# gduguey/DiffUS

Measured on NVIDIA B200. Metric: bmode_frames_per_s_fwd_bwd, higher is better.
Workload: dtype f32

## Files before the change

### diffus_b200/csrc/common.cuh

```cuda
#pragma once
#include <cuda_runtime.h>
#include <stdint.h>
#include <float.h>

#include "../../include/diffus_b200.h"

namespace diffus {

constexpr unsigned FULL = 0xffffffffu;

template <int CH, int CK = 2>
struct Geo {
    static constexpr int CHUNK = CH;
    static constexpr int CKPT = CK;
    static constexpr int SEG = 32 * CH;
    __device__ __forceinline__ static int pad(int i) { return i + (i >> 5); }
    static constexpr int ZBUF = (SEG + 2) + (SEG + 2) / 32 + 3;
    static constexpr int OBUF = (SEG + 1) + (SEG + 1) / 32 + 3;
};
using FwdGeo = Geo<16>;
using BwdGeo = Geo<8, 2>;
constexpr int PREFIX_STRIDE = FwdGeo::SEG;

struct M2 {
    float2 c0, c1;
    __device__ __forceinline__ float a() const { return c0.x; }
    __device__ __forceinline__ float b() const { return c1.x; }
    __device__ __forceinline__ float c() const { return c0.y; }
    __device__ __forceinline__ float d() const { return c1.y; }
};
__device__ __forceinline__ float2 bcast(float s) { return make_float2(s, s); }
__device__ __forceinline__ M2 m2_make(float a, float b, float c, float d) { return M2{make_float2(a, c), make_float2(b, d)}; }
__device__ __forceinline__ M2 m2_identity() { return m2_make(1.f, 0.f, 0.f, 1.f); }
__device__ __forceinline__ M2 m2_zero() { return m2_make(0.f, 0.f, 0.f, 0.f); }
__device__ __forceinline__ M2 m2_mul(const M2& x, const M2& y) {
    return M2{__ffma2_rn(x.c0, bcast(y.c0.x), __fmul2_rn(x.c1, bcast(y.c0.y))),
              __ffma2_rn(x.c0, bcast(y.c1.x), __fmul2_rn(x.c1, bcast(y.c1.y)))};
}
__device__ __forceinline__ M2 m2_mul_interface(const M2& p, float r) {
    float q = __fmaf_rn(-2.f * r, r, 1.f);
    return M2{__ffma2_rn(p.c0, bcast(q), __fmul2_rn(p.c1, bcast(-r))), __ffma2_rn(p.c0, bcast(r), p.c1)};
}
__device__ __forceinline__ M2 m2_mul_interface_t(const M2& x, float r) {
    float q = __fmaf_rn(-2.f * r, r, 1.f);
    return M2{__ffma2_rn(x.c0, bcast(q), __fmul2_rn(x.c1, bcast(r))), __ffma2_rn(x.c0, bcast(-r), x.c1)};
}
__device__ __forceinline__ M2 m2_transpose(const M2& x) { return m2_make(x.a(), x.c(), x.b(), x.d()); }
__device__ __forceinline__ M2 m2_add(const M2& x, const M2& y) { return M2{__fadd2_rn(x.c0, y.c0), __fadd2_rn(x.c1, y.c1)}; }
__device__ __forceinline__ float2 shfl_up2(float2 v, int d) { return make_float2(__shfl_up_sync(FULL, v.x, d), __shfl_up_sync(FULL, v.y, d)); }
__device__ __forceinline__ float2 shfl_down2(float2 v, int d) { return make_float2(__shfl_down_sync(FULL, v.x, d), __shfl_down_sync(FULL, v.y, d)); }
__device__ __forceinline__ float2 shfl2(float2 v, int src) { return make_float2(__shfl_sync(FULL, v.x, src), __shfl_sync(FULL, v.y, src)); }
__device__ __forceinline__ M2 m2_shfl_up(const M2& x, int d) { return M2{shfl_up2(x.c0, d), shfl_up2(x.c1, d)}; }
__device__ __forceinline__ M2 m2_shfl_down(const M2& x, int d) { return M2{shfl_down2(x.c0, d), shfl_down2(x.c1, d)}; }
__device__ __forceinline__ M2 m2_shfl(const M2& x, int src) { return M2{shfl2(x.c0, src), shfl2(x.c1, src)}; }

__device__ __forceinline__ float nan_to_num(float e) {
    if (e != e) return 0.f;
    return fminf(fmaxf(e, -FLT_MAX), FLT_MAX);
}

__device__ __forceinline__ float warp_sum(float v) {
#pragma unroll
    for (int d = 16; d > 0; d >>= 1) v += __shfl_xor_sync(FULL, v, d);
    return v;
}

__device__ __forceinline__ int warp_sum8_index(int lane) { return ((lane & 1) << 2) | (lane & 2) | ((lane >> 2) & 1); }
__device__ __forceinline__ float warp_sum8(float v[8], int lane) {
    const bool b0 = lane & 1, b1 = lane & 2, b2 = lane & 4;
#pragma unroll
    for (int j = 0; j < 4; ++j) {
        const float send = b0 ? v[j] : v[j + 4], keep = b0 ? v[j + 4] : v[j];
        v[j] = keep + __shfl_xor_sync(FULL, send, 1);
    }
#pragma unroll
    for (int j = 0; j < 2; ++j) {
        const float send = b1 ? v[j] : v[j + 2], keep = b1 ? v[j + 2] : v[j];
        v[j] = keep + __shfl_xor_sync(FULL, send, 2);
    }
    const float send = b2 ? v[0] : v[1], keep = b2 ? v[1] : v[0];
    float t = keep + __shfl_xor_sync(FULL, send, 4);
    t += __shfl_xor_sync(FULL, t, 8);
    t += __shfl_xor_sync(FULL, t, 16);
    return t;
}

struct VolumeView {
    const float* data;
    int D, H, W;
    uint32_t sx, sy;
    uint32_t gsx, gsy;
};

constexpr int BRICK_I = 4, BRICK_J = 4, BRICK_K = 2;
constexpr int QUAD_B = 2;

template <int LAYOUT>
struct GradLayout {
    static constexpr int value = (LAYOUT == DIFFUS_LAYOUT_QUAD || LAYOUT == DIFFUS_LAYOUT_TEXTURE) ? DIFFUS_LAYOUT_BRICK : LAYOUT;
};

__device__ __forceinline__ cudaTextureObject_t volume_texture(const void* data) { return (cudaTextureObject_t)(uintptr_t)data; }
__device__ __forceinline__ float4 tex_gather_face(cudaTextureObject_t tex, int layer, float x, float y) {
    float4 r;
    asm volatile("tld4.r.a2d.v4.f32.f32 {%0, %1, %2, %3}, [%4, {%5, %6, %7, %7}];"
                 : "=f"(r.x), "=f"(r.y), "=f"(r.z), "=f"(r.w)
                 : "l"(tex), "r"(layer), "f"(x), "f"(y)
                 : "memory");
    return r;
}
__device__ __forceinline__ float tex_fetch_voxel(cudaTextureObject_t tex, int i, int j, int k) {
    return tex2DLayered<float>(tex, (float)k + 0.5f, (float)j + 0.5f, i);
}

template <int LAYOUT>
__device__ __forceinline__ uint32_t axis_x(uint32_t sx, int i) {
    if (LAYOUT == DIFFUS_LAYOUT_LINEAR) return (uint32_t)i * sx;
    if (LAYOUT == DIFFUS_LAYOUT_BRICK) return (uint32_t)(i >> 2) * sx + ((uint32_t)(i & 3) << 3);
    return (uint32_t)(i >> 1) * sx + (uint32_t)(i & 1);
}
template <int LAYOUT>
__device__ __forceinline__ uint32_t axis_y(uint32_t sy, int j) {
    if (LAYOUT == DIFFUS_LAYOUT_LINEAR) return (uint32_t)j * sy;
    if (LAYOUT == DIFFUS_LAYOUT_BRICK) return (uint32_t)(j >> 2) * sy + ((uint32_t)(j & 3) << 1);
    return (uint32_t)(j >> 1) * sy + ((uint32_t)(j & 1) << 2);
}
template <int LAYOUT>
__device__ __forceinline__ uint32_t axis_z(int k) {
    if (LAYOUT == DIFFUS_LAYOUT_LINEAR) return (uint32_t)k;
    if (LAYOUT == DIFFUS_LAYOUT_BRICK) return ((uint32_t)(k >> 1) << 5) + (uint32_t)(k & 1);
    return ((uint32_t)(k >> 1) << 3) + ((uint32_t)(k & 1) << 1);
}
template <int LAYOUT>
__device__ __forceinline__ uint32_t voxel_offset(const VolumeView& v, int i, int j, int k) {
    return axis_x<LAYOUT>(v.sx, i) + axis_y<LAYOUT>(v.sy, j) + axis_z<LAYOUT>(k);
}

template <int LAYOUT>
__device__ __forceinline__ uint32_t grad_offset(const VolumeView& v, int i, int j, int k) {
    constexpr int GL = GradLayout<LAYOUT>::value;
    return axis_x<GL>(v.gsx, i) + axis_y<GL>(v.gsy, j) + axis_z<GL>(k);
}

__device__ __forceinline__ float fast_rcp(float b) {
    float r;
    asm("rcp.approx.ftz.f32 %0, %1;" : "=f"(r) : "f"(b));
    return r;
}
__device__ __forceinline__ float fast_div(float a, float b) { return a * fast_rcp(b); }
__device__ __forceinline__ float echo_of(float pb, float inv_pd) { return __fmul_rn(pb, inv_pd); }

template <bool POSE64>
struct RaySetup;

template <>
struct RaySetup<false> {
    float s[3], d[3];
    __device__ __forceinline__ void load(const void* src, const void* dir, int64_t pose, int64_t ray,
                                         int64_t n_rays, int64_t dir_pose_stride, int) {
        const float* sp = (const float*)src + pose * 3;
        const float* dp = (const float*)dir + pose * dir_pose_stride + ray * 3;
#pragma unroll
        for (int a = 0; a < 3; ++a) { s[a] = __ldg(sp + a); d[a] = __ldg(dp + a); }
    }
    __device__ __forceinline__ float coord(int a, int k) const {
        return __fadd_rn(s[a], __fmul_rn((float)k, d[a]));
    }
};

template <>
struct RaySetup<true> {
    double s[3], d[3];
    int product_f32;
    __device__ __forceinline__ void load(const void* src, const void* dir, int64_t pose, int64_t ray,
                                         int64_t n_rays, int64_t dir_pose_stride, int prod_f32) {
        const double* sp = (const double*)src + pose * 3;
        const double* dp = (const double*)dir + pose * dir_pose_stride + ray * 3;
#pragma unroll
        for (int a = 0; a < 3; ++a) { s[a] = __ldg(sp + a); d[a] = __ldg(dp + a); }
        product_f32 = prod_f32;
    }
    __device__ __forceinline__ float coord(int a, int k) const {
        double prod = product_f32 ? (double)__fmul_rn((float)k, (float)d[a]) : __dmul_rn((double)k, d[a]);
        return (float)__dadd_rn(s[a], prod);
    }
};

__device__ __forceinline__ int nearest_index(float p, int n) {
    int i = __float2int_rn(p);
    return min(max(i, 0), n - 1);
}

struct TriCell {
    int i0[3], i1[3];
    float f[3];
};

template <bool COLLAPSE = false>
__device__ __forceinline__ void tri_axis(float p, int n, int& i0, int& i1, float& f) {
    float hi = (float)(n - 1);
    float pc = fminf(fmaxf(p, 0.f), hi);
    float fl = floorf(pc);
    f = pc - fl;
    i0 = (int)fl;
    i1 = min(i0 + 1, n - 1);
    if (COLLAPSE) i1 = (p > 0.f) ? i1 : i0;
}

template <bool COLLAPSE>
__device__ __forceinline__ void tri_axis_tex(float p, int n, float& coord, float& f) {
    (void)n;
    const float fl = floorf(p);
    f = p - fl;
    coord = fl + 1.0f;
    if (COLLAPSE) coord = (p > 0.f) ? coord : 0.f;
}

__device__ __forceinline__ bool tri_inside(float f) { return (__float_as_uint(f) >> 31) == 0u; }
__device__ __forceinline__ void tri_axis_flag(float p, int n, int& i0, float& f) {
    float hi = (float)(n - 1);
    float pc = fminf(fmaxf(p, 0.f), hi);
    float fl = floorf(pc);
    f = (p > 0.f) ? pc - fl : -0.f;
    i0 = (int)fl;
}

template <int GLAYOUT>
__device__ __forceinline__ void tri_offsets(const VolumeView& v, const TriCell& c, uint32_t off[8]) {
    uint32_t x0 = axis_x<GLAYOUT>(v.gsx, c.i0[0]), x1 = axis_x<GLAYOUT>(v.gsx, c.i1[0]);
    uint32_t y0 = axis_y<GLAYOUT>(v.gsy, c.i0[1]), y1 = axis_y<GLAYOUT>(v.gsy, c.i1[1]);
    uint32_t z0 = axis_z<GLAYOUT>(c.i0[2]), z1 = axis_z<GLAYOUT>(c.i1[2]);
    uint32_t a00 = x0 + y0, a01 = x0 + y1, a10 = x1 + y0, a11 = x1 + y1;
    off[0] = a00 + z0; off[1] = a00 + z1; off[2] = a01 + z0; off[3] = a01 + z1;
    off[4] = a10 + z0; off[5] = a10 + z1; off[6] = a11 + z0; off[7] = a11 + z1;
}

template <bool GRAD, bool FLAGS = false>
// ... 117 lines not shown
```

### diffus_b200/csrc/render_kernels.cu

```cuda
#include <cuda_pipeline.h>

#include <type_traits>

#include "common.cuh"
#include "launch.h"

namespace diffus {


__device__ __forceinline__ M2 warp_exclusive_prefix(const M2& chunk_total, const M2& carry, int lane) {
    M2 inc = chunk_total;
#pragma unroll
    for (int d = 1; d < 32; d <<= 1) {
        M2 left = m2_shfl_up(inc, d);
        if (lane >= d) inc = m2_mul(left, inc);
    }
    M2 exc = m2_shfl_up(inc, 1);
    if (lane == 0) exc = m2_identity();
    return m2_mul(carry, exc);
}

template <class G>
__device__ __forceinline__ M2 forward_chunk(const float r[G::CHUNK], M2 carry, float* obuf, int lane) {
    M2 T = m2_identity();
#pragma unroll
    for (int i = 0; i < G::CHUNK; ++i) T = m2_mul_interface(T, r[i]);
    M2 P = warp_exclusive_prefix(T, carry, lane);
#pragma unroll
    for (int i = 0; i < G::CHUNK; ++i) {
        P = m2_mul_interface(P, r[i]);
        obuf[G::pad(lane * G::CHUNK) + i] = nan_to_num(echo_of(P.b(), fast_rcp(P.d())));
    }
    return m2_shfl(P, 31);
}

constexpr int LOSS_GRAD = 0, LOSS_MSE = 1;
constexpr int WIDE_CTAS = 4;
constexpr int FWD_GB = 1;
constexpr int TEX_GB = 2;
constexpr int TEX_GB_WIDE = 4;
constexpr int BWD_DZ_STRIDE = FwdGeo::OBUF;

struct ZTail {
    const float* zbuf;
    const float* dz;
    int lane_col;
    float kbase;
    unsigned skip_mask;
    float* rbar1;
    float w_after;
    float w_first;
    float2 acc[3];
    float* xch;
};

struct CoopXch {
    static constexpr int TOTAL = 0;
    static constexpr int MAP_A = 16;
    static constexpr int MAP_B = 32;
    static constexpr int W_FIRST = 48;
    static constexpr int OUT = 52;
    static constexpr int FLOATS = 96;
};
__device__ __forceinline__ void xch_store(float* x, const M2& m) { x[0] = m.a(); x[1] = m.b(); x[2] = m.c(); x[3] = m.d(); }
__device__ __forceinline__ M2 xch_load(const float* x) { return m2_make(x[0], x[1], x[2], x[3]); }

template <class G_, int LOSS, bool ZMODE = false, bool POSE_GRAD = false, bool STORE_ZBAR = false, bool FULL = false,
          bool COOP = false>
__device__ __forceinline__ M2 backward_chunk(const float r[G_::CHUNK], const M2& carry, const M2& vin, float* gbuf,
                                             const float* att_lane, float* frame_lane, float grad_scale, int ncol_lane,
                                             float& loss_acc, int lane, ZTail* zt = nullptr,
                                             const M2* known_total = nullptr, const M2* known_prefix = nullptr,
                                             const float* att_scale = nullptr) {
    constexpr int CHUNK = G_::CHUNK;
    static_assert(!COOP || ZMODE, "COOP: render kernels only");
    const int base = G_::pad(lane * CHUNK);
    M2 T, P;
    if (known_total) {
        T = *known_total;
        P = *known_prefix;
    } else {
        T = m2_identity();
#pragma unroll
        for (int i = 0; i < CHUNK; ++i) T = m2_mul_interface(T, r[i]);
        P = warp_exclusive_prefix(T, carry, lane);
    }
    constexpr int CK = G_::CKPT;
    M2 Pck[CHUNK / CK];
    M2 G = m2_identity();
    M2 B = m2_zero();
#pragma unroll
    for (int i = 0; i < CHUNK; ++i) {
        if (i % CK == 0) Pck[i / CK] = P;
        P = m2_mul_interface(P, r[i]);
        G = m2_mul_interface(G, r[i]);
        float inv = fast_rcp(P.d());
        float e = echo_of(P.b(), inv);
        bool finite = fabsf(e) <= FLT_MAX;
        float ge;
        const float att = att_lane ? (att_scale ? __fmul_rn(att_lane[i], *att_scale) : att_lane[i]) : 1.f;
        if (LOSS == LOSS_MSE) {
            float fr = __fmul_rn(nan_to_num(e), att);
            float diff = fr - gbuf[base + i];
            if (FULL || i < ncol_lane) {
                loss_acc += diff * diff;
                if (frame_lane) frame_lane[i] = fr;
            }
            ge = grad_scale * diff * att;
        } else {
            ge = gbuf[base + i] * att;
        }
        if (!finite || (!FULL && i >= ncol_lane)) ge = 0.f;
        gbuf[base + i] = ge;
        const float2 dcol = make_float2(ge * inv, -ge * e * inv);
        B.c0 = __ffma2_rn(dcol, bcast(G.b()), B.c0);
        B.c1 = __ffma2_rn(dcol, bcast(G.d()), B.c1);
    }
    M2 As = m2_transpose(T), Bs = B;
#pragma unroll
    for (int d = 1; d < 32; d <<= 1) {
        M2 An = m2_shfl_down(As, d), Bn = m2_shfl_down(Bs, d);
        if (lane + d < 32) {
            Bs = m2_add(m2_mul(Bn, As), Bs);
            As = m2_mul(An, As);
        }
    }
    M2 An = m2_shfl_down(As, 1), Bn = m2_shfl_down(Bs, 1);
    M2 vin_ = vin;
    if (COOP) {
        const int w = threadIdx.x >> 5;
        if (lane == 0) {
            xch_store(zt->xch + CoopXch::MAP_A + 4 * w, As);
            xch_store(zt->xch + CoopXch::MAP_B + 4 * w, Bs);
        }
        __syncthreads();
        vin_ = m2_zero();
        for (int u = (int)(blockDim.x >> 5) - 1; u > w; --u)
            vin_ = m2_add(m2_mul(vin_, xch_load(zt->xch + CoopXch::MAP_A + 4 * u)), xch_load(zt->xch + CoopXch::MAP_B + 4 * u));
    }
    M2 V = (lane == 31) ? vin_ : m2_add(m2_mul(vin_, An), Bn);
    M2 vout = m2_add(m2_mul(vin_, As), Bs);
    const float* zl = nullptr;
    const float* dzl = nullptr;
    float z_hh = 0.f, z_hi = 0.f, w_prev = 0.f, part_last = 0.f, z_after = 0.f;
    if (ZMODE) {
        zl = zt->zbuf + G_::pad(zt->lane_col);
        if (POSE_GRAD) dzl = zt->dz + G_::pad(zt->lane_col);
        z_hi = zt->zbuf[G_::pad(zt->lane_col + CHUNK)];
        z_hh = zt->zbuf[G_::pad(zt->lane_col + CHUNK + 1)];
        z_after = z_hh;
    }
    auto emit = [&](int i, float zbar) {
        if (!(zbar == zbar) || (!FULL && i >= ncol_lane)) zbar = 0.f;
        if (STORE_ZBAR) gbuf[base + i] = zbar;
// ... 457 lines not shown
                    int idx = (t0 + u) * 32 + lane;
                    if (idx < ncol) {
                        float g[3];
                        float z = fe[u].template finish<POSE_GRAD>(g);
                        zbuf[G::pad(idx + 1)] = z;
                        if (POSE_GRAD) {
                            const int di = G::pad(idx);
                            dz[di] = g[0]; dz[BWD_DZ + di] = g[1]; dz[2 * BWD_DZ + di] = g[2];
                        }
                    } else if (POSE_GRAD) {
                        const int di = G::pad(idx);
                        dz[di] = 0.f; dz[BWD_DZ + di] = 0.f; dz[2 * BWD_DZ + di] = 0.f;
                    }
                }
            }
            __pipeline_wait_prior(0);
        }
        if (COOP) {
            __syncthreads();
            if (lane == 0 && warp > 0) zbuf[G::pad(0)] = zbuf[G::pad(SS) - BWD_SMEM_PER_WARP];
        }
        if (lane == 0) {
            if (s > 0 && !COOP) {
                int k = p.start + c0 - 1;
                float g[3];
                zbuf[G::pad(0)] = sample_volume<SAMPLER, LAYOUT, false>(p.vol, rs.coord(0, k), rs.coord(1, k), rs.coord(2, k), g);
            }
            if (!COOP) zbuf[G::pad(ncol + 1)] = carry_z;
        }
        __syncwarp();

        M2 carry[BWD_SUB];
        carry[0] = m2_identity();
        if (!COOP && s > 0) {
            float4 c4 = __ldg((const float4*)(p.seg_prefix + (ray * p.nprefix + (s - 1)) * 4));
            carry[0] = m2_make(c4.x, c4.y, c4.z, c4.w);
        }
        float r[G::CHUNK];
        M2 T0 = m2_identity(), E0 = m2_identity();
        static_assert(BWD_SUB <= 2, "the prefix pass keeps one sub-segment's products in registers");
        static_assert(!COOP || BWD_SUB == 1, "COOP: one sub-segment per pass");
        const bool have0 = BWD_SUB == 2 && nsub > 1;
        const bool coop_full = COOP && p.Sout == (int)(blockDim.x >> 5) * SS;
        if (COOP) {
            if (ncol == SS) chunk_reflections<G, true>(zbuf, c0, ncol, p.median, med, lane, r, 0);
            else chunk_reflections<G, false>(zbuf, c0, ncol, p.median, med, lane, r, 0);
#pragma unroll
            for (int i = 0; i < G::CHUNK; ++i) T0 = m2_mul_interface(T0, r[i]);
            const M2 el = warp_exclusive_prefix(T0, m2_identity(), lane);
            const M2 tot = m2_shfl(m2_mul(el, T0), 31);
            if (lane == 0) xch_store(zt.xch + CoopXch::TOTAL + 4 * warp, tot);
            __syncthreads();
            for (int u = 0; u < warp; ++u) carry[0] = m2_mul(carry[0], xch_load(zt.xch + CoopXch::TOTAL + 4 * u));
            E0 = m2_mul(carry[0], el);
            if (lane == 0) zbuf[G::pad(ncol + 1)] = warp + 1 < (int)(blockDim.x >> 5) ? zbuf[BWD_SMEM_PER_WARP + G::pad(1)] : 0.f;
            __syncwarp();
        } else if (BWD_SUB == 1) {
        } else if (have0) {
            chunk_reflections<G, true>(zbuf, c0, ncol, p.median, med, lane, r, 0);
#pragma unroll
            for (int i = 0; i < G::CHUNK; ++i) T0 = m2_mul_interface(T0, r[i]);
            E0 = warp_exclusive_prefix(T0, carry[0], lane);
            carry[BWD_SUB - 1] = m2_shfl(m2_mul(E0, T0), 31);
        } else {
            carry[BWD_SUB - 1] = carry[0];
        }
        zt.w_after = (c0 + ncol < p.Sout) ? carry_w : 0.f;
#pragma unroll
        for (int h = BWD_SUB - 1; h >= 0; --h) {
            if (h < nsub) {
                const int off = h * G::SEG;
                const bool full = COOP ? coop_full : ncol - off >= G::SEG;
                if (COOP) {
                } else if (full) chunk_reflections<G, true>(zbuf, c0, ncol, p.median, med, lane, r, off);
                else chunk_reflections<G, false>(zbuf, c0, ncol, p.median, med, lane, r, off);
                const int lane_col = off + lane * G::CHUNK;
                zt.skip_mask = 0u;
                if (c0 + lane_col == 0) zt.skip_mask = p.median ? 3u : 1u;
                zt.lane_col = lane_col;
                zt.kbase = (float)(p.start + c0 + lane_col);
                zt.rbar1 = (p.first_rbar && s == 0 && h == 0) ? p.first_rbar + ray : nullptr;
                const M2* kt = (COOP || (h == 0 && have0)) ? &T0 : nullptr;
                M2 ch = carry[0];
                if (BWD_SUB == 2 && h == 1) ch = carry[BWD_SUB - 1];
                float* fl = fout ? fout + c0 + lane_col : nullptr;
                float* gl = gbuf + G::pad(off);
                const float pass_scale = ONE_PASS ? 1.f : expf(-p.alpha * (float)c0);
                const float* asc = ONE_PASS ? nullptr : &pass_scale;
                if (full)
                    vin = backward_chunk<G, LOSS, true, POSE_GRAD, VOL_GRAD, true, COOP>(
                        r, ch, vin, gl, att + G::pad(ONE_PASS ? c0 + lane_col : lane_col), fl, p.grad_scale, ncol - lane_col,
                        loss_acc, lane, &zt, kt, &E0, asc);
                else
                    vin = backward_chunk<G, LOSS, true, POSE_GRAD, VOL_GRAD, false, COOP>(
                        r, ch, vin, gl, att + G::pad(ONE_PASS ? c0 + lane_col : lane_col), fl, p.grad_scale, ncol - lane_col,
                        loss_acc, lane, &zt, kt, &E0, asc);
                zt.w_after = zt.w_first;
            }
        }
        carry_w = zt.w_first;
        carry_z = zbuf[G::pad(1)];
        __syncwarp();

        if (VOL_GRAD) {
            if (GradLayout<LAYOUT>::value == DIFFUS_LAYOUT_BRICK) {
                scatter_pass_quads<SAMPLER, POSE64>(p, rs, gbuf, c0, ncol, lane);
            } else {
                for (int t = 0; t < ntile; ++t) {
                    int idx = t * 32 + lane;
                    if (idx < ncol) {
                        float zbar = gbuf[G::pad(idx)];
                        if (zbar != 0.f) scatter_volume_grad<SAMPLER, LAYOUT, POSE64>(p, rs, p.start + c0 + idx, zbar);
                    }
                }
            }
            __syncwarp();
        }
    }
    if (COOP) {
        float* out = zt.xch + CoopXch::OUT + 8 * warp;
        {
            float v[8] = {zt.acc[0].x, zt.acc[1].x, zt.acc[2].x, zt.acc[0].y, zt.acc[1].y, zt.acc[2].y, loss_acc, 0.f};
            const float t = warp_sum8(v, lane);
            if (lane < 8) out[warp_sum8_index(lane)] = t;
        }
        __syncthreads();
        if (warp == 0 && lane < 7) {
            const float* o = zt.xch + CoopXch::OUT + lane;
            float v = o[0];
            for (int u = 1; u < (int)(blockDim.x >> 5); ++u) v += o[8 * u];
            if (POSE_GRAD && lane < 3) p.grad_src_partial[ray * 3 + lane] = v;
            if (POSE_GRAD && lane >= 3 && lane < 6) p.grad_dir[ray * 3 + lane - 3] = v;
            if (LOSS == LOSS_MSE && lane == 6 && p.loss_partial) p.loss_partial[ray] = v;
        }
        return;
    }
    if (POSE_GRAD) {
        float v[8] = {zt.acc[0].x, zt.acc[1].x, zt.acc[2].x, zt.acc[0].y, zt.acc[1].y, zt.acc[2].y, loss_acc, 0.f};
        const float t = warp_sum8(v, lane);
        const int j = warp_sum8_index(lane);
        if (lane < 8) {
            if (j < 3) p.grad_src_partial[ray * 3 + j] = t;
            else if (j < 6) p.grad_dir[ray * 3 + j - 3] = t;
            else if (j == 6 && LOSS == LOSS_MSE && p.loss_partial) p.loss_partial[ray] = t;
        }
        return;
    }
    if (LOSS == LOSS_MSE && p.loss_partial) {
        float l = warp_sum(loss_acc);
        if (lane == 0) p.loss_partial[ray] = l;
    }
}

#ifndef DIFFUS_LAYOUT_SLICE
__global__ void __launch_bounds__(128) echo_fwd_kernel(const float* __restrict__ refl, int64_t n_rays, int N,
                                                       float* __restrict__ echo) {
    using G = FwdGeo;
    extern __shared__ __align__(16) float smem[];
    const int warp = threadIdx.x >> 5, lane = threadIdx.x & 31;
    const int64_t ray = (int64_t)blockIdx.x * (blockDim.x >> 5) + warp;
    if (ray >= n_rays) return;
    float* rbuf = smem + warp * (2 * G::OBUF);
    float* obuf = rbuf + G::OBUF;
    const int Sout = N + 1, nseg = (Sout + G::SEG - 1) / G::SEG;
    const float* rin = refl + ray * (int64_t)N;
    float* out = echo + ray * (int64_t)Sout;
    M2 carry = m2_identity();
    for (int s = 0; s < nseg; ++s) {
        const int c0 = s * G::SEG, ncol = min(G::SEG, Sout - c0);
        for (int idx = lane; idx < G::SEG; idx += 32) {
            int c = c0 + idx;
            rbuf[G::pad(idx)] = (c >= 1 && idx < ncol) ? __ldg(rin + c - 1) : 0.f;
        }
        __syncwarp();
        float r[G::CHUNK];
#pragma unroll
        for (int i = 0; i < G::CHUNK; ++i) r[i] = rbuf[G::pad(lane * G::CHUNK + i)];
        carry = forward_chunk<G>(r, carry, obuf, lane);
        __syncwarp();
        for (int idx = lane; idx < ncol; idx += 32) out[c0 + idx] = obuf[G::pad(idx)];
        __syncwarp();
    }
}

__global__ void __launch_bounds__(128) echo_bwd_kernel(const float* __restrict__ refl, const float* __restrict__ grad_echo,
                                                       int64_t n_rays, int N, float* __restrict__ grad_refl) {
    using G = BwdGeo;
    extern __shared__ __align__(16) float smem[];
    const int warp = threadIdx.x >> 5, lane = threadIdx.x & 31;
    const int64_t ray = (int64_t)blockIdx.x * (blockDim.x >> 5) + warp;
    if (ray >= n_rays) return;
    const int Sout = N + 1, nseg = (Sout + G::SEG - 1) / G::SEG;
    float* rbuf = smem + warp * (2 * G::OBUF + 4 * nseg);
    float* gbuf = rbuf + G::OBUF;
    float* prefix = gbuf + G::OBUF;
    const float* rin = refl + ray * (int64_t)N;
    const float* gin = grad_echo + ray * (int64_t)Sout;
    float* gout = grad_refl + ray * (int64_t)N;
    M2 carry = m2_identity();
    for (int s = 0; s < nseg; ++s) {
        const int c0 = s * G::SEG, ncol = min(G::SEG, Sout - c0);
        if (lane == 0) { prefix[4 * s] = carry.a(); prefix[4 * s + 1] = carry.b(); prefix[4 * s + 2] = carry.c(); prefix[4 * s + 3] = carry.d(); }
        if (s + 1 == nseg) break;
        for (int idx = lane; idx < G::SEG; idx += 32) {
            int c = c0 + idx;
            rbuf[G::pad(idx)] = (c >= 1 && idx < ncol) ? __ldg(rin + c - 1) : 0.f;
        }
        __syncwarp();
        M2 T = m2_identity();
#pragma unroll
        for (int i = 0; i < G::CHUNK; ++i) T = m2_mul_interface(T, rbuf[G::pad(lane * G::CHUNK + i)]);
        M2 P = warp_exclusive_prefix(T, carry, lane);
        carry = m2_shfl(m2_mul(P, T), 31);
        __syncwarp();
    }
    __syncwarp();
    M2 vin = m2_zero();
    float unused = 0.f;
    for (int s = nseg - 1; s >= 0; --s) {
        const int c0 = s * G::SEG, ncol = min(G::SEG, Sout - c0);
        for (int idx = lane; idx < G::SEG; idx += 32) {
            int c = c0 + idx;
            bool ok = idx < ncol;
            rbuf[G::pad(idx)] = (c >= 1 && ok) ? __ldg(rin + c - 1) : 0.f;
            gbuf[G::pad(idx)] = ok ? __ldg(gin + c) : 0.f;
        }
        __syncwarp();
        float r[G::CHUNK];
#pragma unroll
        for (int i = 0; i < G::CHUNK; ++i) r[i] = rbuf[G::pad(lane * G::CHUNK + i)];
        M2 cs = m2_make(prefix[4 * s], prefix[4 * s + 1], prefix[4 * s + 2], prefix[4 * s + 3]);
        vin = backward_chunk<G, LOSS_GRAD>(r, cs, vin, gbuf, nullptr, nullptr, 0.f, ncol - lane * G::CHUNK, unused, lane);
        __syncwarp();
        for (int idx = lane; idx < ncol; idx += 32) {
            int c = c0 + idx;
            if (c >= 1) gout[c - 1] = gbuf[G::pad(idx)];
        }
        __syncwarp();
    }
}

__device__ __forceinline__ double block_sum_fixed_order(double acc, double* warp_part) {
#pragma unroll
    for (int d = 16; d > 0; d >>= 1) acc += __shfl_xor_sync(FULL, acc, d);
    if ((threadIdx.x & 31) == 0) warp_part[threadIdx.x >> 5] = acc;
    __syncthreads();
    double t = 0.0;
    if (threadIdx.x == 0)
        for (int w = 0; w < (int)(blockDim.x >> 5); ++w) t += warp_part[w];
    return t;
}

__device__ __forceinline__ double sum_partials(const float* __restrict__ x, int64_t n) {
    double a0 = 0.0, a1 = 0.0, a2 = 0.0, a3 = 0.0;
    const int64_t n4 = ((((uintptr_t)x) & 15u) == 0) ? n >> 2 : 0;
    const float4* x4 = (const float4*)x;
#pragma unroll 4
    for (int64_t i = threadIdx.x; i < n4; i += blockDim.x) {
        const float4 v = __ldg(x4 + i);
        a0 += (double)v.x; a1 += (double)v.y; a2 += (double)v.z; a3 += (double)v.w;
    }
    for (int64_t i = (n4 << 2) + threadIdx.x; i < n; i += blockDim.x) a0 += (double)__ldg(x + i);
    return (a0 + a1) + (a2 + a3);
}

__global__ void __launch_bounds__(1024) reduce_sum_kernel(const float* __restrict__ partial, int64_t n, float scale,
                                                          float* __restrict__ out, double* __restrict__ block_sums) {
    __shared__ double warp_part[32];
    const int64_t per = ((n + gridDim.x - 1) / gridDim.x + 3) & ~(int64_t)3;
    const int64_t lo = min(n, (int64_t)blockIdx.x * per), hi = min(n, lo + per);
    const double acc = sum_partials(partial + lo, hi - lo);
    const double t = block_sum_fixed_order(acc, warp_part);
    if (threadIdx.x == 0) {
        if (block_sums) block_sums[blockIdx.x] = t;
        else out[0] = (float)(t * (double)scale);
    }
}

__global__ void reduce_final_kernel(const double* __restrict__ block_sums, int n, float scale, float* __restrict__ out) {
    if (threadIdx.x == 0) {
        double t = 0.0;
        for (int b = 0; b < n; ++b) t += block_sums[b];
        out[0] = (float)(t * (double)scale);
    }
}

__global__ void __launch_bounds__(1024) reduce_rays_and_sum_kernel(const float* __restrict__ src_partial, int64_t n_poses, int64_t n_rays,
                                                                   float* __restrict__ grad_src, const float* __restrict__ loss_partial,
                                                                   int64_t n, float scale, float* __restrict__ loss_out) {
    __shared__ double warp_part[32];
    if (blockIdx.x == gridDim.x - 1) {
        const double t = block_sum_fixed_order(sum_partials(loss_partial, n), warp_part);
        if (threadIdx.x == 0) loss_out[0] = (float)(t * (double)scale);
        return;
    }
    const int warp = threadIdx.x >> 5, lane = threadIdx.x & 31;
    const int64_t pose = (int64_t)blockIdx.x * 32 + warp;
    if (pose >= n_poses) return;
    float a0 = 0.f, a1 = 0.f, a2 = 0.f;
    const float* src = src_partial + pose * n_rays * 3;
    for (int64_t r = lane; r < n_rays; r += 32) { a0 += src[r * 3]; a1 += src[r * 3 + 1]; a2 += src[r * 3 + 2]; }
    a0 = warp_sum(a0); a1 = warp_sum(a1); a2 = warp_sum(a2);
    if (lane == 0) { grad_src[pose * 3] = a0; grad_src[pose * 3 + 1] = a1; grad_src[pose * 3 + 2] = a2; }
}

bool reduce_rays_and_sum_fits(int64_t n) { return n <= ((int64_t)1 << 18); }

cudaError_t launch_reduce_rays_and_sum(const float* src_partial, int64_t n_poses, int64_t n_rays, float* grad_src,
                                       const float* loss_partial, int64_t n, float scale, float* loss_out, cudaStream_t st) {
    const unsigned grid = (unsigned)((n_poses + 31) / 32) + 1u;
    reduce_rays_and_sum_kernel<<<grid, 1024, 0, st>>>(src_partial, n_poses, n_rays, grad_src, loss_partial, n, scale, loss_out);
    return cudaGetLastError();
}

constexpr int REDUCE_BLOCKS = 64;
int64_t reduce_sum_workspace_bytes() { return REDUCE_BLOCKS * sizeof(double); }

cudaError_t launch_reduce_sum(const float* partial, int64_t n, float scale, float* out, void* workspace, cudaStream_t st) {
    if (n <= ((int64_t)1 << 18)) {
        reduce_sum_kernel<<<1, 1024, 0, st>>>(partial, n, scale, out, nullptr);
        return cudaGetLastError();
    }
    double* sums = (double*)workspace;
    reduce_sum_kernel<<<REDUCE_BLOCKS, 1024, 0, st>>>(partial, n, scale, out, sums);
    reduce_final_kernel<<<1, 32, 0, st>>>(sums, REDUCE_BLOCKS, scale, out);
    return cudaGetLastError();
}

#endif

static int warps_per_block(int64_t total_rays) {
    if (total_rays >= 4 * 148 * 4) return 4;
    if (total_rays >= 2 * 148 * 2) return 2;
    return 1;
}

#ifdef DIFFUS_LAYOUT_SLICE
#define DIFFUS_CAT2(a, b) a##b
#define DIFFUS_CAT(a, b) DIFFUS_CAT2(a, b)
#define DIFFUS_FWD_NAME DIFFUS_CAT(launch_render_fwd_layout, DIFFUS_LAYOUT_SLICE)
#define DIFFUS_BWD_NAME DIFFUS_CAT(launch_render_bwd_layout, DIFFUS_LAYOUT_SLICE)

cudaError_t DIFFUS_FWD_NAME(const RenderParams& p_in, int sampler, int layout, int pose64, cudaStream_t st) {
    RenderParams p = p_in;
    if (!p.frame) p.att_slots = 0;
    int wpb = warps_per_block(p.total_rays);
    size_t smem = ((size_t)p.att_slots + (size_t)wpb * FWD_SMEM_PER_WARP) * sizeof(float);
    unsigned grid = (unsigned)((p.total_rays + wpb - 1) / wpb);
    DIFFUS_DISPATCH(auto k = render_fwd_kernel<S_, L_, P64_>; cudaError_t e = ensure_smem(k, smem, 28 / wpb);
                    if (e != cudaSuccess) return e; k<<<grid, wpb * 32, smem, st>>>(p); return cudaGetLastError())
    return cudaErrorInvalidValue;
}

template <int S_, int L_, bool P64_, int LOSS>
static cudaError_t launch_bwd_g(const RenderParams& p, bool pg, bool vg, unsigned grid, int threads, size_t smem,
                                cudaStream_t st) {
    constexpr bool TRI = S_ == DIFFUS_SAMPLER_TRILINEAR;
#define DIFFUS_BWD_GO(PG, VG)                                                                                         \
    {                                                                                                                 \
           \
                                                        \
        constexpr bool WIDE_ = !P64_ && ((TRI && PG && !VG) || (VG && !PG && LOSS == LOSS_MSE));                      \
        constexpr bool COOP_ = !P64_ && TRI && PG && !VG;                                                             \
        if (WIDE_ && p.Sout <= PREFIX_STRIDE && p.Sout > BwdGeo::SEG) {                                               \
            auto k = render_bwd_kernel<S_, L_, false, PG, VG, LOSS, true, WIDE_>;                                     \
            cudaError_t e = ensure_smem(k, smem, WIDE_CTAS * 4 / (threads / 32));                                     \
            if (e != cudaSuccess) return e;                                                                           \
            k<<<grid, threads, smem, st>>>(p);                                                                        \
            return cudaGetLastError();                                                                                \
        }                                                                                                             \
        if (!P64_ && p.Sout <= PREFIX_STRIDE) {                                                                       \
            auto k = render_bwd_kernel<S_, L_, false, PG, VG, LOSS, true>;                                            \
            cudaError_t e = ensure_smem(k, smem, ((VG) ? 16 : 20) / (threads / 32));                                  \
            if (e != cudaSuccess) return e;                                                                           \
            k<<<grid, threads, smem, st>>>(p);                                                                        \
            return cudaGetLastError();                                                                                \
        }                                                                                                             \
        if (render_bwd_is_coop(p.Sout, p.total_rays, S_, P64_, PG, VG)) {  \
            auto k = render_bwd_kernel<S_, L_, false, PG, VG, LOSS, false, COOP_, COOP_>;                             \
            const int nw_ = (p.Sout + PREFIX_STRIDE - 1) / PREFIX_STRIDE;        \
            const size_t smem_ = ((size_t)p.att_slots_padded + (size_t)nw_ * BWD_SMEM_PER_WARP + CoopXch::FLOATS) * sizeof(float); \
            cudaError_t e = ensure_smem(k, smem_, 16 / nw_);                                                          \
            if (e != cudaSuccess) return e;                                                                           \
            k<<<(unsigned)p.total_rays, nw_ * 32, smem_, st>>>(p);                                                    \
            return cudaGetLastError();                                                                                \
        }                                                                                                             \
        auto k = render_bwd_kernel<S_, L_, P64_, PG, VG, LOSS, false>;                                                \
        cudaError_t e = ensure_smem(k, smem, 16 / (threads / 32));                                                    \
        if (e != cudaSuccess) return e;                                                                               \
        k<<<grid, threads, smem, st>>>(p);                                                                            \
        return cudaGetLastError();                                                                                    \
    }
    if (!TRI) pg = false;
    if (pg && vg) DIFFUS_BWD_GO(TRI, true)
    if (pg) DIFFUS_BWD_GO(TRI, false)
    if (vg) DIFFUS_BWD_GO(false, true)
    DIFFUS_BWD_GO(false, false)
#undef DIFFUS_BWD_GO
}

cudaError_t DIFFUS_BWD_NAME(const RenderParams& p, int sampler, int layout, int pose64, bool pose_grad, bool vol_grad,
                            cudaStream_t st) {
    int wpb = warps_per_block(p.total_rays);
    size_t smem = ((size_t)p.att_slots_padded + (size_t)wpb * BWD_SMEM_PER_WARP) * sizeof(float);
    unsigned grid = (unsigned)((p.total_rays + wpb - 1) / wpb);
    const bool mse = p.target != nullptr;
    DIFFUS_DISPATCH(if (mse) return launch_bwd_g<S_, L_, P64_, LOSS_MSE>(p, pose_grad, vol_grad, grid, wpb * 32, smem, st);
                    return launch_bwd_g<S_, L_, P64_, LOSS_GRAD>(p, pose_grad, vol_grad, grid, wpb * 32, smem, st))
    return cudaErrorInvalidValue;
}

#else

cudaError_t launch_render_fwd(const RenderParams& p, int sampler, int layout, int pose64, cudaStream_t st) {
    switch (layout) {
        case DIFFUS_LAYOUT_LINEAR: return launch_render_fwd_layout0(p, sampler, layout, pose64, st);
        case DIFFUS_LAYOUT_BRICK: return launch_render_fwd_layout1(p, sampler, layout, pose64, st);
        case DIFFUS_LAYOUT_QUAD: return launch_render_fwd_layout2(p, sampler, layout, pose64, st);
        case DIFFUS_LAYOUT_TEXTURE: return launch_render_fwd_layout3(p, sampler, layout, pose64, st);
    }
    return cudaErrorInvalidValue;
}

cudaError_t launch_render_bwd(const RenderParams& p, int sampler, int layout, int pose64, bool pose_grad, bool vol_grad,
                              cudaStream_t st) {
    switch (layout) {
        case DIFFUS_LAYOUT_LINEAR: return launch_render_bwd_layout0(p, sampler, layout, pose64, pose_grad, vol_grad, st);
        case DIFFUS_LAYOUT_BRICK: return launch_render_bwd_layout1(p, sampler, layout, pose64, pose_grad, vol_grad, st);
        case DIFFUS_LAYOUT_QUAD: return launch_render_bwd_layout2(p, sampler, layout, pose64, pose_grad, vol_grad, st);
        case DIFFUS_LAYOUT_TEXTURE: return launch_render_bwd_layout3(p, sampler, layout, pose64, pose_grad, vol_grad, st);
    }
    return cudaErrorInvalidValue;
}

cudaError_t launch_echo_fwd(const float* refl, int64_t n_rays, int N, float* echo, cudaStream_t st) {
    int wpb = warps_per_block(n_rays);
    size_t smem = (size_t)wpb * 2 * FwdGeo::OBUF * sizeof(float);
    echo_fwd_kernel<<<(unsigned)((n_rays + wpb - 1) / wpb), wpb * 32, smem, st>>>(refl, n_rays, N, echo);
    return cudaGetLastError();
}

cudaError_t launch_echo_bwd(const float* refl, const float* grad_echo, int64_t n_rays, int N, float* grad_refl,
                            cudaStream_t st) {
    int wpb = warps_per_block(n_rays);
    int nseg = (N + 1 + BwdGeo::SEG - 1) / BwdGeo::SEG;
    size_t smem = (size_t)wpb * (2 * BwdGeo::OBUF + 4 * nseg) * sizeof(float);
    cudaError_t e = ensure_smem(echo_bwd_kernel, smem);
    if (e != cudaSuccess) return e;
    echo_bwd_kernel<<<(unsigned)((n_rays + wpb - 1) / wpb), wpb * 32, smem, st>>>(refl, grad_echo, n_rays, N, grad_refl);
    return cudaGetLastError();
}
#endif

}
```

Baseline: 2.009 million.

## Add warp-specialized pose-gradient backward kernel with mbarrier producer/consumer ring

Adds a persistent warp-specialized backward kernel for the texture/trilinear pose-gradient MSE path. Gather warps load targets and texture samples into a shared-memory ring, while sweep warps run the backward scan, synchronized through mbarriers. setmaxnreg shifts registers from the gather warpgroups to the sweep warpgroups. The goal is to overlap texture fetch latency with the compute-heavy sweep, at the cost of one CTA per SM, a fixed split between warp roles, and more complex synchronization.

```diff
diff --git a/diffus_b200/csrc/common.cuh b/diffus_b200/csrc/common.cuh
--- a/diffus_b200/csrc/common.cuh
+++ b/diffus_b200/csrc/common.cuh
@@ -83,6 +83,27 @@
     t += __shfl_xor_sync(FULL, t, 8);
     t += __shfl_xor_sync(FULL, t, 16);
     return t;
+}
+
+template <int N>
+__device__ __forceinline__ void setmaxnreg_dec() { asm volatile("setmaxnreg.dec.sync.aligned.u32 %0;" ::"n"(N)); }
+template <int N>
+__device__ __forceinline__ void setmaxnreg_inc() { asm volatile("setmaxnreg.inc.sync.aligned.u32 %0;" ::"n"(N)); }
+
+__device__ __forceinline__ void mbar_init(uint64_t* bar, unsigned count) {
+    asm volatile("mbarrier.init.shared::cta.b64 [%0], %1;" ::"r"((uint32_t)__cvta_generic_to_shared(bar)), "r"(count) : "memory");
+}
+__device__ __forceinline__ void mbar_arrive(uint64_t* bar) {
+    asm volatile("mbarrier.arrive.shared::cta.b64 _, [%0];" ::"r"((uint32_t)__cvta_generic_to_shared(bar)) : "memory");
+}
+__device__ __forceinline__ void mbar_wait(uint64_t* bar, unsigned parity) {
+    asm volatile(
+        "{\n\t.reg .pred done;\n"
+        "WAIT:\n\t"
+        "mbarrier.try_wait.parity.shared::cta.b64 done, [%0], %1;\n\t"
+        "@!done bra WAIT;\n}" ::"r"((uint32_t)__cvta_generic_to_shared(bar)),
+        "r"(parity)
+        : "memory");
 }
 
 struct VolumeView {
diff --git a/diffus_b200/csrc/render_kernels.cu b/diffus_b200/csrc/render_kernels.cu
--- a/diffus_b200/csrc/render_kernels.cu
+++ b/diffus_b200/csrc/render_kernels.cu
@@ -1,5 +1,6 @@
 #include <cuda_pipeline.h>
 
+#include <algorithm>
 #include <type_traits>
 
 #include "common.cuh"
@@ -763,6 +764,200 @@
     }
 }
 
+#if defined(DIFFUS_LAYOUT_SLICE) && DIFFUS_LAYOUT_SLICE == DIFFUS_LAYOUT_TEXTURE
+#ifndef DIFFUS_WS_GW
+#define DIFFUS_WS_GW 12
+#endif
+constexpr int WS_GATHER_WARPS = DIFFUS_WS_GW;
+constexpr int WS_SWEEP_WARPS = 8;
+constexpr int WS_SLOTS = 2 * WS_SWEEP_WARPS;
+constexpr int WS_THREADS = 32 * (WS_GATHER_WARPS + WS_SWEEP_WARPS);
+constexpr int WS_LAUNCH_REGS = 65536 / WS_THREADS / 8 * 8;
+#ifndef DIFFUS_WS_GREGS
+#define DIFFUS_WS_GREGS 48
+#define DIFFUS_WS_SREGS 168
+#endif
+#ifndef DIFFUS_WS_GB
+#define DIFFUS_WS_GB 2
+#endif
+constexpr int WS_GATHER_REGS = DIFFUS_WS_GREGS;
+constexpr int WS_SWEEP_REGS = DIFFUS_WS_SREGS;
+constexpr int WS_GB = DIFFUS_WS_GB;
+constexpr int WS_HEAD = 4 * WS_SLOTS + WS_SLOTS;
+static_assert((WideGeo::SEG / 32) % WS_GB == 0, "the tail batches must not run past the last tile of the buffers");
+static_assert(WS_GATHER_WARPS % 4 == 0 && WS_SWEEP_WARPS % 4 == 0, "setmaxnreg acts on whole warpgroups");
+static_assert(WS_GATHER_WARPS * WS_GATHER_REGS + WS_SWEEP_WARPS * WS_SWEEP_REGS <= (WS_THREADS / 32) * WS_LAUNCH_REGS,
+              "setmaxnreg.inc would wait forever: the pool is the CTA's launch allocation");
+
+__global__ void __launch_bounds__(WS_THREADS, 1) render_pose_ws_kernel(const RenderParams p) {
+    using G = WideGeo;
+    constexpr int SAMPLER = DIFFUS_SAMPLER_TRILINEAR, LAYOUT = DIFFUS_LAYOUT_TEXTURE;
+    extern __shared__ __align__(16) float smem[];
+    uint64_t* full = (uint64_t*)smem;
+    uint64_t* empty = full + WS_SLOTS;
+    float* slot_med = smem + 4 * WS_SLOTS;
+    float* att = smem + WS_HEAD;
+    float* ring = att + p.att_slots_padded;
+    const int warp = threadIdx.x >> 5, lane = threadIdx.x & 31;
+    const int64_t per = p.total_rays / gridDim.x, extra = p.total_rays % gridDim.x;
+    const int64_t ray0 = (int64_t)blockIdx.x * per + min((int64_t)blockIdx.x, extra);
+    const int nray = (int)(per + ((int64_t)blockIdx.x < extra ? 1 : 0));
+    const int ncol = p.Sout;
+    if (threadIdx.x < WS_SLOTS) {
+        mbar_init(full + threadIdx.x, 32);
+        mbar_init(empty + threadIdx.x, 32);
+    }
+    fill_attenuation_padded<G>(att, ncol, p.alpha);
+
+    if (warp < WS_GATHER_WARPS) {
+        setmaxnreg_dec<WS_GATHER_REGS>();
+        const uint64_t stream_policy = l2_evict_first_policy();
+        const int lane_z = lane + 1 + (lane == 31 ? 1 : 0);
+        for (int j = warp; j < nray; j += WS_GATHER_WARPS) {
+            const int s = j % WS_SLOTS, u = j / WS_SLOTS;
+#if DIFFUS_WS_MODE == 2
+            if (u > 0) break;
+#endif
+            const int64_t ray = ray0 + j;
+            const int64_t pose = pose_of_ray(ray, p);
+            RaySetup<false> rs;
+            rs.load(p.sources, p.directions, pose, ray - pose * p.n_rays, p.n_rays, p.dir_pose_stride, p.product_f32);
+            const float med = p.median ? __ldg(p.median + pose) : 0.f;
+            float* zbuf = ring + s * BWD_SMEM_PER_WARP;
+            float* gbuf = zbuf + BWD_ZBUF;
+            float* dz = gbuf + BWD_OBUF;
+            const float* gin = p.target + ray * (int64_t)ncol;
+            if (u > 0) mbar_wait(empty + s, (u - 1) & 1);
+            {
+                const int nfull = ncol >> 5;
+                if (nfull == G::SEG / 32) {
+#pragma unroll
+                    for (int t = 0; t < G::SEG / 32; ++t) cp_async_stream4(gbuf + lane + 33 * t, gin + lane + 32 * t, stream_policy);
+                } else {
+                    for (int t = 0; t < nfull; ++t) cp_async_stream4(gbuf + lane + 33 * t, gin + lane + 32 * t, stream_policy);
+                }
+                for (int t = nfull; t < G::SEG / 32; ++t) {
+                    const int idx = t * 32 + lane;
+                    if (idx < ncol) cp_async_stream4(gbuf + G::pad(idx), gin + idx, stream_policy);
+                    else gbuf[G::pad(idx)] = 0.f;
+                }
+                __pipeline_commit();
+            }
+            const int nt_full = (ncol >> 5) / WS_GB * WS_GB;
+            for (int t0 = 0; t0 < nt_full; t0 += WS_GB) {
+                Fetch<SAMPLER, LAYOUT> fe[WS_GB];
+#pragma unroll
+                for (int u2 = 0; u2 < WS_GB; ++u2) {
+                    const int k = p.start + (t0 + u2) * 32 + lane;
+                    fe[u2].template issue<true>(p.vol, rs.coord(0, k), rs.coord(1, k), rs.coord(2, k));
+                }
+                float* zt0 = zbuf + 33 * t0 + lane_z;
+                float* dt0 = dz + 33 * t0 + lane;
+#pragma unroll
+                for (int u2 = 0; u2 < WS_GB; ++u2) {
+                    float g[3];
+                    zt0[33 * u2] = fe[u2].template finish<true>(g);
+                    dt0[33 * u2] = g[0]; dt0[BWD_DZ + 33 * u2] = g[1]; dt0[2 * BWD_DZ + 33 * u2] = g[2];
+                }
+            }
+            for (int t0 = nt_full; t0 < G::SEG / 32; t0 += WS_GB) {
+                Fetch<SAMPLER, LAYOUT> fe[WS_GB];
+#pragma unroll
+                for (int u2 = 0; u2 < WS_GB; ++u2) {
+                    const int idx = (t0 + u2) * 32 + lane;
+                    if (idx < ncol) {
+                        const int k = p.start + idx;
+                        fe[u2].template issue<true>(p.vol, rs.coord(0, k), rs.coord(1, k), rs.coord(2, k));
+                    }
+                }
+#pragma unroll
+                for (int u2 = 0; u2 < WS_GB; ++u2) {
+                    const int idx = (t0 + u2) * 32 + lane;
+                    const int di = G::pad(idx);
+                    if (idx < ncol) {
+                        float g[3];
+                        zbuf[G::pad(idx + 1)] = fe[u2].template finish<true>(g);
+                        dz[di] = g[0]; dz[BWD_DZ + di] = g[1]; dz[2 * BWD_DZ + di] = g[2];
+                    } else {
+                        dz[di] = 0.f; dz[BWD_DZ + di] = 0.f; dz[2 * BWD_DZ + di] = 0.f;
+                    }
+                }
+            }
+            if (lane == 0) {
+                zbuf[0] = 0.f;
+                zbuf[G::pad(ncol + 1)] = 0.f;
+                slot_med[s] = med;
+            }
+            __pipeline_wait_prior(0);
+            mbar_arrive(full + s);
+        }
+        return;
+    }
+
+    setmaxnreg_inc<WS_SWEEP_REGS>();
+    const int lane_col = lane * G::CHUNK;
+    for (int j = warp - WS_GATHER_WARPS; j < nray; j += WS_SWEEP_WARPS) {
+        const int s = j % WS_SLOTS, u = j / WS_SLOTS;
+        const int64_t ray = ray0 + j;
+        float* zbuf = ring + s * BWD_SMEM_PER_WARP;
+        float* gbuf = zbuf + BWD_ZBUF;
+        ZTail zt;
+        zt.zbuf = zbuf;
+        zt.dz = gbuf + BWD_OBUF;
+        zt.lane_col = lane_col;
+        zt.kbase = (float)(p.start + lane_col);
+        zt.skip_mask = lane == 0 ? (p.median ? 3u : 1u) : 0u;
+        zt.rbar1 = p.first_rbar ? p.first_rbar + ray : nullptr;
+        zt.w_after = 0.f;
+        zt.xch = nullptr;
+#pragma unroll
+        for (int a = 0; a < 3; ++a) zt.acc[a] = make_float2(0.f, 0.f);
+        float loss_acc = 0.f;
+        float* fl = p.frame ? p.frame + ray * (int64_t)ncol + lane_col : nullptr;
+        float r[G::CHUNK];
+#if DIFFUS_WS_MODE == 2
+        if (u == 0)
+#endif
+        mbar_wait(full + s, u & 1);
+#if DIFFUS_WS_MODE == 1
+        mbar_arrive(empty + s);
+        continue;
+#endif
+        const float med = slot_med[s];
+        if (ncol == G::SEG) {
+            chunk_reflections<G, true>(zbuf, 0, ncol, p.median, med, lane, r, 0);
+            backward_chunk<G, LOSS_MSE, true, true, false, true>(r, m2_identity(), m2_zero(), gbuf, att + G::pad(lane_col), fl,
+                                                                 p.grad_scale, ncol - lane_col, loss_acc, lane, &zt);
+        } else {
+            chunk_reflections<G, false>(zbuf, 0, ncol, p.median, med, lane, r, 0);
+            backward_chunk<G, LOSS_MSE, true, true, false, false>(r, m2_identity(), m2_zero(), gbuf, att + G::pad(lane_col), fl,
+                                                                  p.grad_scale, ncol - lane_col, loss_acc, lane, &zt);
+        }
+        mbar_arrive(empty + s);
+        float v[8] = {zt.acc[0].x, zt.acc[1].x, zt.acc[2].x, zt.acc[0].y, zt.acc[1].y, zt.acc[2].y, loss_acc, 0.f};
+        const float t = warp_sum8(v, lane);
+        const int i = warp_sum8_index(lane);
+        if (lane < 8) {
+            if (i < 3) p.grad_src_partial[ray * 3 + i] = t;
+            else if (i < 6) p.grad_dir[ray * 3 + i - 3] = t;
+            else if (i == 6 && p.loss_partial) p.loss_partial[ray] = t;
+        }
+    }
+}
+
+cudaError_t launch_pose_ws(const RenderParams& p, cudaStream_t st) {
+    int dev = 0, sms = 0;
+    cudaError_t e = cudaGetDevice(&dev);
+    if (e == cudaSuccess) e = cudaDeviceGetAttribute(&sms, cudaDevAttrMultiProcessorCount, dev);
+    if (e != cudaSuccess) return e;
+    const size_t smem = ((size_t)WS_HEAD + (size_t)p.att_slots_padded + (size_t)WS_SLOTS * BWD_SMEM_PER_WARP) * sizeof(float);
+    e = ensure_smem(render_pose_ws_kernel, smem, 1);
+    if (e != cudaSuccess) return e;
+    render_pose_ws_kernel<<<(unsigned)std::min<int64_t>(sms, p.total_rays), WS_THREADS, smem, st>>>(p);
+    return cudaGetLastError();
+}
+#endif
+
 #ifndef DIFFUS_LAYOUT_SLICE
 __global__ void __launch_bounds__(128) echo_fwd_kernel(const float* __restrict__ refl, int64_t n_rays, int N,
                                                        float* __restrict__ echo) {
@@ -963,6 +1158,9 @@
     return cudaErrorInvalidValue;
 }
 
+cudaError_t launch_pose_ws(const RenderParams& p, cudaStream_t st);
+constexpr int64_t WS_MIN_RAYS = 1;
+
 template <int S_, int L_, bool P64_, int LOSS>
 static cudaError_t launch_bwd_g(const RenderParams& p, bool pg, bool vg, unsigned grid, int threads, size_t smem,
                                 cudaStream_t st) {
@@ -973,6 +1171,11 @@
                                                         \
         constexpr bool WIDE_ = !P64_ && ((TRI && PG && !VG) || (VG && !PG && LOSS == LOSS_MSE));                      \
         constexpr bool COOP_ = !P64_ && TRI && PG && !VG;                                                             \
+                          \
+        if constexpr (L_ == DIFFUS_LAYOUT_TEXTURE && !P64_ && TRI && PG && !VG && LOSS == LOSS_MSE) {                    \
+            if (p.Sout <= PREFIX_STRIDE && p.Sout > BwdGeo::SEG && p.total_rays >= WS_MIN_RAYS)                       \
+                return launch_pose_ws(p, st);                                                                         \
+        }                                                                                                             \
         if (WIDE_ && p.Sout <= PREFIX_STRIDE && p.Sout > BwdGeo::SEG) {                                               \
             auto k = render_bwd_kernel<S_, L_, false, PG, VG, LOSS, true, WIDE_>;                                     \
             cudaError_t e = ensure_smem(k, smem, WIDE_CTAS * 4 / (threads / 32));                                     \
```

After: 1.667 million, median of 6. 17.0% lower.
